# synthesizer-project/synference

Hardware: AMD Instinct MI355X
Metric: posterior samples/sec (accepted, prior-box rejection included) (higher is better)
Workload: dtype f32

## Files before the change

include/synference_hip.h:

```cpp
#ifndef SYNFERENCE_HIP_H
#define SYNFERENCE_HIP_H

#include <stddef.h>
#include <stdint.h>

#ifdef __cplusplus
extern "C" {
#endif

typedef struct sf_flow sf_flow;
typedef struct sf_opt sf_opt;

enum sf_status {
  SF_OK = 0,
  SF_ERR_INVALID = -1,
  SF_ERR_HIP = -2,
  SF_ERR_NO_DEVICE = -3,
  SF_ERR_STATE = -4
};

enum sf_kind { SF_MAF = 0, SF_NSF = 1, SF_NSF_AR = 2, SF_MAF_AR = 3 };

typedef struct sf_flow_desc {
  int32_t kind;
// ... 23 lines not shown
void sf_flow_destroy(sf_flow* f);
int64_t sf_flow_num_params(const sf_flow* f);
int64_t sf_flow_packed_size(const sf_flow* f);

int sf_flow_set_params(sf_flow* f, const float* flat, int64_t n, int is_device, void* stream);

int sf_flow_get_params(sf_flow* f, float* flat, int64_t n, int is_device, void* stream);

int sf_flow_pack_table(const sf_flow* f, int32_t* src1, int32_t* src2, int64_t n_packed);
int64_t sf_flow_packed16_size(const sf_flow* f);
int sf_flow_pack_table16(const sf_flow* f, int32_t* src1, int32_t* src2, int64_t n_packed16);
int64_t sf_flow_packed16b_size(const sf_flow* f);
int sf_flow_pack_table16b(const sf_flow* f, int32_t* src, int64_t n);
int64_t sf_flow_packed16c_size(const sf_flow* f);
int sf_flow_pack_table16c(const sf_flow* f, int32_t* src, int64_t n);
int64_t sf_flow_trainc_size(const sf_flow* f);
int64_t sf_flow_trainc_grad_size(const sf_flow* f);
int sf_flow_trainc_table(const sf_flow* f, int32_t* src1, int32_t* src2, int64_t n, int32_t* gdst, int64_t n_params,
                         int32_t* desc , float* cst, int64_t n_cst);
int64_t sf_flow_cst_size(const sf_flow* f);
int sf_flow_train_path(const sf_flow* f, int64_t B, int want_dctx);
int sf_flow_describe(const sf_flow* f, char* buf, size_t buflen);

int sf_flow_log_prob(sf_flow* f, const float* theta , const float* x ,
                     int64_t B, float* out , void* stream);

int sf_flow_log_prob_grad(sf_flow* f, const float* theta , const float* x, int64_t rows_per_x, int64_t B,
                          float* lp , float* dtheta , void* stream);

int sf_map_step(int64_t B, int64_t D, float* phi , float* exp_avg , float* exp_avg_sq ,
// ... 272 lines not shown
```

synference_amd/_lib.py:

```python
from __future__ import annotations

import ctypes as C
import os
from pathlib import Path

_HERE = Path(__file__).resolve().parent
LIB_PATH = _HERE / "lib" / "libsynference_hip.so"

c_f32p = C.POINTER(C.c_float)
c_i32p = C.POINTER(C.c_int32)
c_u32p = C.POINTER(C.c_uint32)


class sf_flow_desc(C.Structure):
    _fields_ = [
        ("kind", C.c_int32), ("D", C.c_int32), ("C", C.c_int32), ("H", C.c_int32),
        ("T", C.c_int32), ("K", C.c_int32), ("NB", C.c_int32), ("scale_fn", C.c_int32),
        ("hidden_bf16", C.c_int32),
        ("tail_bound", C.c_float), ("min_bin_width", C.c_float), ("min_bin_height", C.c_float),
        ("min_derivative", C.c_float), ("maf_eps", C.c_float), ("lu_eps", C.c_float),
        ("theta_mean", c_f32p), ("theta_std", c_f32p), ("x_mean", c_f32p), ("x_std", c_f32p),
        ("perms", c_i32p), ("ar_slope", C.c_float),
    ]

# ... 69 lines not shown
    "sf_flow_packed16_size": (C.c_int64, [C.c_void_p]),
    "sf_flow_pack_table16": (C.c_int, [C.c_void_p, C.c_void_p, C.c_void_p, C.c_int64]),
    "sf_flow_packed16b_size": (C.c_int64, [C.c_void_p]),
    "sf_flow_inverse_from_noise_sampler": (C.c_int, [C.c_void_p, C.c_void_p, C.c_void_p, C.c_int64, C.c_void_p, C.c_void_p]),
    "sf_set_sampler_fp32": (C.c_int, [C.c_int]),
    "sf_flow_set_sample_row_offset": (C.c_int, [C.c_void_p, C.c_int64]),
    "sf_flow_train_path": (C.c_int, [C.c_void_p, C.c_int64, C.c_int]),
    "sf_flow_trainc_size": (C.c_int64, [C.c_void_p]),
    "sf_flow_trainc_grad_size": (C.c_int64, [C.c_void_p]),
    "sf_flow_cst_size": (C.c_int64, [C.c_void_p]),
    "sf_flow_trainc_table": (C.c_int, [C.c_void_p, C.c_void_p, C.c_void_p, C.c_int64, C.c_void_p, C.c_int64, C.c_void_p,
                                       C.c_void_p, C.c_int64]),
    "sf_flow_pack_table16b": (C.c_int, [C.c_void_p, C.c_void_p, C.c_int64]),
    "sf_flow_packed16c_size": (C.c_int64, [C.c_void_p]),
    "sf_flow_pack_table16c": (C.c_int, [C.c_void_p, C.c_void_p, C.c_int64]),
    "sf_flow_get_params": (C.c_int, [C.c_void_p, C.c_void_p, C.c_int64, C.c_int, C.c_void_p]),
    "sf_flow_prepare_context": (C.c_int, [C.c_void_p, C.c_void_p, C.c_int64, C.c_void_p]),
    "sf_flow_release_context": (C.c_int, [C.c_void_p]),
    "sf_flow_sample": (C.c_int, [C.c_void_p, C.c_void_p, C.c_int64, C.c_int64, C.c_void_p, C.c_void_p,
                                 C.c_uint64, C.c_int32, C.c_void_p, C.c_void_p, C.POINTER(C.c_int64),
                                 C.c_void_p]),
    "sf_flow_sample_slots": (C.c_int, [C.c_void_p, C.c_void_p, C.c_int64, C.c_int64, C.c_void_p, C.c_int64, C.c_void_p,
                                       C.c_void_p, C.c_uint64, C.c_int32, C.c_void_p, C.POINTER(C.c_int64), C.c_void_p]),
    "sf_flow_sample_stats": (C.c_int, [C.c_void_p, C.POINTER(C.c_float)]),
    "sf_flow_acceptance": (C.c_int, [C.c_void_p, C.c_void_p, C.c_int64, C.c_int64, C.c_void_p, C.c_void_p,
                                     C.c_uint64, C.c_void_p, C.c_void_p]),
    "sf_flow_loss_grad": (C.c_int, [C.c_void_p, C.c_void_p, C.c_void_p, C.c_void_p, C.c_int64, C.c_float,
                                    C.c_void_p, C.c_void_p, C.c_void_p]),
    "sf_flow_loss_grad_rows": (C.c_int, [C.c_void_p, C.c_void_p, C.c_void_p, C.c_void_p, C.c_void_p, C.c_int64,
                                         C.c_float, C.c_void_p, C.c_void_p, C.c_void_p, C.c_void_p, C.c_void_p,
# ... 92 lines not shown
```

synference_amd/csrc/sf_api.hip:

```cpp
#include <hip/hip_runtime.h>

#include <chrono>
#include <cmath>
#include <cstdio>
#include <cstdlib>
#include <cstring>
#include <string>
#include <vector>

#include "sf_internal.h"
#include "sf_train.h"
#include "sf_nsf1.h"
#include "sf_nsfar.h"
#include "sf_nsfc.h"
#include "sf_trainc.h"

namespace {
thread_local std::string g_err;

int hip_fail(hipError_t e, const char* what) {
  return sf_fail(SF_ERR_HIP, std::string(what) + ": " + hipGetErrorString(e));
}
}

// ... 14 lines not shown
  SF_TRY_SET(hipMemset(d.d_packed, 0, np * sizeof(float)));
  SF_TRY_SET(d.d_cst.upload(f->L.cst));
  SF_TRY_SET(d.d_s1.alloc(np));
  SF_TRY_SET(d.d_s2.alloc(np));
  SF_TRY_SET(hipMemcpy(d.d_s1, f->L.src1.data(), np * sizeof(int32_t), hipMemcpyHostToDevice));
  SF_TRY_SET(hipMemcpy(d.d_s2, f->L.src2.data(), np * sizeof(int32_t), hipMemcpyHostToDevice));
  if ((f->L.dev.m16_ok || f->L.nsfS.ok) && f->L.n_packed16 > 0) {
    const size_t n16 = (size_t)f->L.n_packed16;
    SF_TRY_SET(d.d_packed16.alloc(n16));
    SF_TRY_SET(d.d_s16a.alloc(n16));
    SF_TRY_SET(d.d_s16b.alloc(n16));
    SF_TRY_SET(hipMemcpy(d.d_s16a, f->L.src16a.data(), n16 * sizeof(int32_t), hipMemcpyHostToDevice));
    SF_TRY_SET(hipMemcpy(d.d_s16b, f->L.src16b.data(), n16 * sizeof(int32_t), hipMemcpyHostToDevice));
  }
  if (f->L.dev.m16_ok && f->L.n_packed16 > 0 && sf_maf16_compact_fix(f->L.dev) == 1) {
    SF_TRY_SET(d.d_packed16c.alloc((size_t)f->L.dev.t16c_stride * f->L.dev.T));
    SF_TRY_SET(d.d_s16c.upload(f->L.src16c));
  }
  if ((f->L.dev.m16_ok || f->L.nsfS.ok) && f->L.n_packed16B > 0) {
    const size_t nB = (size_t)f->L.n_packed16B;
    SF_TRY_SET(d.d_packed16B.alloc(nB));
    SF_TRY_SET(d.d_s16B.alloc(nB));
    SF_TRY_SET(hipMemcpy(d.d_s16B, f->L.src16B.data(), nB * sizeof(int32_t), hipMemcpyHostToDevice));
  }
  if (f->L.n_packedB > 0) {
    SF_TRY_SET(d.d_packedB.alloc((size_t)f->L.n_packedB));
    SF_TRY_SET(d.d_bsrc.alloc((size_t)f->L.n_packedB));
    SF_TRY_SET(hipMemcpy(d.d_bsrc, f->L.srcB.data(), (size_t)f->L.n_packedB * sizeof(int32_t), hipMemcpyHostToDevice));
  }
  SF_TRY_SET(d.d_flat.alloc((size_t)f->L.n_params));
  SF_TRY_SET(d.d_cnt.alloc(SF_MAX_ROUNDS));
  SF_TRY_SET(d.h_cnt.alloc(SF_MAX_ROUNDS));
// ... 94 lines not shown
int64_t sf_flow_packed16b_size(const sf_flow* f) { return (f && f->L.dev.m16_ok) ? f->L.n_packed16B : 0; }

int sf_flow_pack_table16b(const sf_flow* f, int32_t* src, int64_t n) {
  if (!f || !src) return sf_fail(SF_ERR_INVALID, "null argument");
  if (!f->L.dev.m16_ok || n != f->L.n_packed16B) return sf_fail(SF_ERR_INVALID, "no split-bf16 image or size mismatch");
  std::memcpy(src, f->L.src16B.data(), (size_t)n * sizeof(int32_t));
  return SF_OK;
}

int64_t sf_flow_packed16c_size(const sf_flow* f) { return (f && f->L.dev.m16_ok) ? (int64_t)f->L.src16c.size() : 0; }

int sf_flow_pack_table16c(const sf_flow* f, int32_t* src, int64_t n) {
  if (!f || !src) return sf_fail(SF_ERR_INVALID, "null argument");
  if (!f->L.dev.m16_ok || n == 0 || n != (int64_t)f->L.src16c.size()) return sf_fail(SF_ERR_INVALID, "no compact fused image or size mismatch");
  std::memcpy(src, f->L.src16c.data(), (size_t)n * sizeof(int32_t));
  return SF_OK;
}

int64_t sf_flow_trainc_size(const sf_flow* f) { return (f && (f->L.trc.ok || f->L.nsc.ok)) ? f->L.n_imgC : 0; }
int64_t sf_flow_trainc_grad_size(const sf_flow* f) { return (f && (f->L.trc.ok || f->L.nsc.ok)) ? f->L.n_gradC : 0; }
int64_t sf_flow_cst_size(const sf_flow* f) { return f ? (int64_t)f->L.cst.size() : 0; }
int sf_flow_trainc_table(const sf_flow* f, int32_t* src1, int32_t* src2, int64_t n, int32_t* gdst, int64_t n_params,
                         int32_t* desc, float* cst, int64_t n_cst) {
  if (!f || !src1 || !src2 || !gdst || !desc || !cst) return sf_fail(SF_ERR_INVALID, "null argument");
  if ((!f->L.trc.ok && !f->L.nsc.ok) || n != f->L.n_imgC || n_params != f->L.n_params || n_cst != (int64_t)f->L.cst.size())
    return sf_fail(SF_ERR_INVALID, "no cooperative training image or size mismatch");
  static_assert(sizeof(SfTrcDev) <= 64 * sizeof(int32_t) && sizeof(SfNscDev) <= 64 * sizeof(int32_t), "descriptor words");
  std::memcpy(src1, f->L.srcC1.data(), (size_t)n * sizeof(int32_t));
  std::memcpy(src2, f->L.srcC2.data(), (size_t)n * sizeof(int32_t));
  std::memcpy(gdst, f->L.gdstC.data(), (size_t)n_params * sizeof(int32_t));
// ... 46 lines not shown
  add("inc_ok", v.inc_ok); add("hidden_bf16", v.hidden_bf16); add("tB_stride", v.tB_stride); add("n_parts", v.n_parts); add("part_max", v.part_max);
  add("n_params", f->L.n_params); add("n_packed", f->L.n_packed);
  {
    int R = 0, NV = 0;
    SfDev vv = v;
    vv.packed16 = reinterpret_cast<const float*>(1);
    sf_ctab_shape(vv, R, NV);
    add("ctab_floats_per_galaxy", (long)v.T * NV * R);
  }
  add("o16_w0", v.o16_w0); add("o16_wc", v.o16_wc); add("o16_b0", v.o16_b0); add("o16_wk0", v.o16_wk[0]);
  add("o16_wk1", v.o16_wk[1]); add("o16_bk0", v.o16_bk[0]); add("o16_bk1", v.o16_bk[1]); add("o16_hv", v.o16_hv);
  add("o16_hvb", v.o16_hvb); add("o16_wh", v.o16_wh); add("o16_bh", v.o16_bh); add("o16_wp", v.o16_wp); add("t16_a_tab", v.t16_a_tab);
  add("t16_a", v.t16_a); add("t16B_stride", v.t16B_stride); add("nP16", v.nP16); add("o16B_wk0", v.o16B_wk[0]); add("o16B_wk1", v.o16B_wk[1]);
  add("t16c_stride", v.t16c_stride); add("o16c_bk1", v.o16c_bk1); add("o16c_hvb", v.o16c_hvb); add("o16c_bh", v.o16c_bh);
  add("o16c_wh", v.o16c_wh); add("o16c_wp", v.o16c_wp); add("o16c_blk", v.o16c_blk); add("c16_fix", sf_maf16_compact_fix(v));
  add("sampler_fused", (f->dev_ready && f->ctab_x) ? (sf_maf16_plan(sampler_dev(f, f->ctab_x)).fused ? 1 : 0) : 0);
  add("m16_ok", v.m16_ok); add("m16_span", v.m16_span); add("m16_k3", v.m16_k3); add("nT16", v.nT16); add("nC16", v.nC16); add("t16_stride", v.t16_stride);
  s += "\"g16_tile\": [";
  for (int i = 0; i < SF_DMAX; ++i) s += std::to_string(v.g16_tile[i]) + (i + 1 < SF_DMAX ? ", " : "], ");
  s += "\"g16_lo\": [";
  for (int i = 0; i < SF_DMAX; ++i) s += std::to_string(v.g16_lo[i]) + (i + 1 < SF_DMAX ? ", " : "], ");
  s += "\"g_kend\": [";
  for (int i = 0; i < SF_DMAX; ++i) s += std::to_string(v.g_kend[i]) + (i + 1 < SF_DMAX ? ", " : "], ");
  s += "\"g_lo\": [";
  for (int i = 0; i < SF_DMAX; ++i) s += std::to_string(v.g_lo[i]) + (i + 1 < SF_DMAX ? ", " : "], ");
  s += "\"g_tile\": [";
  for (int i = 0; i < SF_DMAX; ++i) s += std::to_string(v.g_tile[i]) + (i + 1 < SF_DMAX ? ", " : "], ");
  s += "\"mt_kend\": [";
  for (int i = 0; i < 4; ++i) s += std::to_string(v.mt_kend[i]) + (i + 1 < 4 ? ", " : "], ");
  s += "\"cst\": [";
// ... 812 lines not shown
```

synference_amd/csrc/sf_layout.cpp:

```cpp
#include "sf_layout.h"

#include <cmath>
#include <cstring>
#include <functional>

namespace {

struct Emitter {
  std::vector<int32_t>& s1;
  std::vector<int32_t>& s2;
  std::vector<int32_t>* gidx = nullptr;
  int64_t cur = 0;

  int64_t pad_to(int64_t align) {
    while (cur % align) push(-1, -1);
    return cur;
  }
  void push(int32_t a, int32_t b, int64_t g = -1) {
    s1.push_back(a);
    s2.push_back(b);
    if (gidx) gidx->push_back((int32_t)(g >= 0 ? g : cur));
    ++cur;
  }
  int64_t linear(int OT, int nG, const std::vector<int>& orow, const std::vector<int>& irow,
// ... 999 lines not shown
    run(v.o16_hvb, 2 * D);
    align(4);
    v.o16c_bh = here();
    run(v.o16_bh, 16);
    v.o16c_wh = here();
    run(v.o16_wh, NT * 256);
    v.o16c_wp = here();
    const int KN = std::min(NT, D - 1);
    run(v.o16_wp, (KN * NT - KN * (KN - 1) / 2) * 16);
    v.o16c_blk = here();
    if (NB == 2)
      for (int ot = 0; ot < NT; ++ot)
        for (int it = 0; it <= ot; ++it) run(v.o16_wk[1] + (ot * NT + it) * 256, 256);
    align(256);
    v.t16c_stride = here();
  }
  L.n_packedB = (int64_t)L.srcB.size();
  {
    const int budget = 152 * 1024 / 4;
    std::vector<int> cuts;
    if (d.kind == SF_MAF) {
      cuts = {0, v.t_stride};
    } else {
      cuts.push_back(0);
      for (int k = 0; k < NB; ++k) cuts.push_back(v.o_wg[k]);
      cuts.push_back(v.o_wout);
      cuts.push_back(v.t_stride);
    }
    v.n_parts = 0;
    v.part_max = 0;
// ... 102 lines not shown
```

synference_amd/csrc/sf_layout.h:

```cpp
#pragma once
#include <cstdint>
#include <string>
#include <vector>

#include "../../include/synference_hip.h"

#define SF_DMAX 16
#define SF_NBMAX 4

struct SfDev {
  const float* packed;
  const float* packedT;
  const float* cst;
  int kind, D, C, H, T, K, NB, scale_fn;
  int HT;
  int PT;
  int KMAX;
  int JP;
  int nGu, nGc, nGh;
  int t_stride;
  int n_parts, part_off[5], part_max;
  int blk_part[SF_NBMAX], head_part;
  int partB_off[5], part_bytes_max;
  int o_w0, o_wc, o_b0;
// ... 15 lines not shown
  int g_tile[SF_DMAX], g_kend[SF_DMAX];
  int g_lo[SF_DMAX];
  int mt_kend[4];
  const unsigned short* packedB;
  int hidden_bf16, nKS, tB_stride;
  int oB_wk[SF_NBMAX], oB_w1[SF_NBMAX], oB_w2[SF_NBMAX];
  const float* packed16;
  int m16_ok, nT16, nC16, t16_stride;
  int t16_a;
  int t16_a_tab;
  int o16_wh, o16_bh;
  int o16_wp;
  const float* packed16c;
  int t16c_stride;
  int o16c_bk1, o16c_hvb, o16c_bh, o16c_wh, o16c_wp, o16c_blk;
  const uint32_t* packed16B;
  int t16B_stride, nP16, o16B_wk[2];
  int m16_span;
  int m16_k3;
  int o16_w0, o16_wc, o16_b0, o16_wk[2], o16_bk[2], o16_hv, o16_hvb;
  int g16_tile[SF_DMAX];
  int g16_lo[SF_DMAX];
  const float* ctab;
  int ctab_R, ctab_NV;
  int c_pscale, c_pshift, c_tdim, c_xmean, c_xstd;
  int c_dslot;
  float logdet0;
  float tail_bound, min_w, min_h, min_d, eps, lu_eps, inv_sqrt_h, deriv_const;
};

// ... 42 lines not shown
  std::vector<int32_t> srcC1, srcC2;
  std::vector<int32_t> gdstC;
  int64_t n_imgC = 0, n_gradC = 0;
  int64_t n_params = 0;
  int64_t n_packed = 0;
  std::vector<int32_t> src1, src2;
  std::vector<int32_t> srcT1, srcT2;
  int64_t n_packedT = 0;
  std::vector<int32_t> gdst;
  std::vector<int32_t> srcB;
  std::vector<int32_t> src16a, src16b;
  std::vector<int32_t> src16B;
  int64_t n_packed16B = 0;
  int64_t n_packed16 = 0;
  std::vector<int32_t> src16c;
  int64_t n_packedB = 0;
  std::vector<float> cst;
  std::string error;
};

static inline int sf_tile_row(int r, int h) { return (r & 3) + 8 * (r >> 2) + 4 * h; }

bool sf_build_layout(const sf_flow_desc& d, SfLayout& L);

#define SF_MLP_LMAX 4
struct SfMlpDev {
  const float* packed;
  const float* packedT;
  const float* cst;
  int n_in, n_out, L, act, HT;
// ... 14 lines not shown
```

synference_amd/csrc/sf_maf16.hip:

```cpp
#include "sf_maf16_pass.h"

template <int NB, bool SPAN>
__global__ __launch_bounds__(256, 3) void k_maf_inv16(SfDev m, SfSampleArgsHost a) {
  const int lane = threadIdx.x & 63, wave = threadIdx.x >> 6;
  const int s = lane & 15, g4 = lane >> 4;
  const long item = ((long)blockIdx.x * 4 + wave) * 16 + s;
  const bool valid = item < a.n_items;
  const long it = valid ? item : a.n_items - 1;
  const SfItem16 I = sf_item16(m, a, it, g4);
  f32x4 u = I.u;
  const uint32_t slot = I.slot, att_mine = I.att;
  const long gal = I.gal, ps_idx = I.ps;
  const float* xr = a.x + gal * m.C;
  float logdet = 0.f;

  const float* ctg = (m.ctab && !a.z_in) ? m.ctab + (size_t)gal * m.T * m.ctab_R : nullptr;
  f32x4 ct0;
  if (!ctg) ct0 = sf_ctx_tile16(m, xr, 0, g4);

  const int NT = m.nT16;
  SfPass16 S;
#pragma unroll
  for (int k = 0; k < 3; ++k)
#pragma unroll
// ... 123 lines not shown
           m.o16_hv == o_hv && m.o16_hvb == o_hvb && m.o16_wh == o_wh && m.o16_bh == o_bh && m.o16_wp == o_wp && m.t16_a_tab == a_tab &&
           m.o16B_wk[0] == 0 && (NB < 2 || m.o16B_wk[1] == oB_wk1) && m.t16B_stride == B_stride;
  }
  static __device__ __forceinline__ void apply(SfDev& m) {
    m.nT16 = NT; m.o16_w0 = o_w0; m.o16_b0 = o_b0; m.o16_bk[0] = o_bk0; m.o16_bk[1] = o_bk1; m.o16_hv = o_hv; m.o16_hvb = o_hvb;
    m.o16_wh = o_wh; m.o16_bh = o_bh; m.o16_wp = o_wp; m.t16_a_tab = a_tab; m.o16B_wk[0] = 0; m.o16B_wk[1] = oB_wk1; m.t16B_stride = B_stride;
  }
};

template <int NB, int DD>
struct SfFixC16 {
  static constexpr int NT = DD - 1, ENT = NT * (NT + 1) / 2;
  static constexpr int o_bk1 = 0, o_hvb = NB == 2 ? NT * 16 : 0, o_bh = o_hvb + (2 * DD + 3) / 4 * 4, o_wh = o_bh + 16;
  static constexpr int o_wp = o_wh + NT * 256, o_blk = o_wp + ENT * 16;
  static constexpr int size = (o_blk + (NB == 2 ? ENT * 256 : 0) + 255) / 256 * 256;
  static constexpr int groups = size / 256;
  static bool matches(const SfDev& m) {
    return m.nT16 == NT && m.o16c_bk1 == o_bk1 && m.o16c_hvb == o_hvb && m.o16c_bh == o_bh && m.o16c_wh == o_wh && m.o16c_wp == o_wp &&
           m.o16c_blk == o_blk && m.t16c_stride == size;
  }
  static __device__ __forceinline__ void apply(SfDev& m) {
    m.o16_bk[1] = o_bk1; m.o16_hvb = o_hvb; m.o16_bh = o_bh; m.o16_wh = o_wh; m.o16_wp = o_wp;
  }
};
template <int PREC>
static __host__ __device__ __forceinline__ int sf_lds_floats16(const SfDev& m, bool cp) {
  if constexpr (PREC == 2) return m.t16c_stride + 4 * SF_G16_SCR;
  else return (m.ctab ? m.t16_a_tab : m.t16_a) + SfHid16<PREC>::lds_floats(m, cp);
}
template <int G>
__device__ __forceinline__ void sf_stage16c(const float* src, int wave) {
  const float4* __restrict__ g = reinterpret_cast<const float4*>(src) + (threadIdx.x & 63);
  float4* __restrict__ l = reinterpret_cast<float4*>(sf_lds16);
  for (int gi = __builtin_amdgcn_readfirstlane(wave); gi < G; gi += 4)
    __builtin_amdgcn_global_load_lds((const void*)(g + gi * 64), (void __attribute__((address_space(3)))*)(l + gi * 64), 16, 0, 0);
  __builtin_amdgcn_s_waitcnt(0x0f70);
}

#ifndef SF_SAMP16_WG_FUSED
#define SF_SAMP16_WG_FUSED 4
#endif
template <int NB, bool SPAN, bool HM, int DD = 0, int PREC = 0, int K3 = 0>
__global__ __launch_bounds__(256, (SPAN ? 3 : (PREC == 2 ? SF_SAMP16_WG_FUSED : 4))) void k_maf_samp16(SfSamp16Args args_in) {
  static_assert(K3 == 0 || (PREC == 2 && K3 <= DD - 1), "skipped k-steps: the fused passes only, at most every hidden tile");
  static_assert(DD == 0 || (HM && !SPAN && DD >= 2 && DD <= 5), "unrolled passes: head tile, aligned placement, D <= 5");
  static_assert(PREC != 2 || DD >= 3, "fused first layer: unrolled kernels only (m_fix and the compact image's offsets)");
  using HID = SfHid16<PREC>;
  constexpr int TPW = SF_SAMP16_TPW;
  constexpr int IPW = 64 * TPW;
  const int wave = threadIdx.x >> 6;
  using FC = SfFixC16<NB, (PREC == 2 ? DD : 2)>;
  unsigned int* ctrl = reinterpret_cast<unsigned int*>(sf_lds16 + sf_lds_floats16<PREC>(args_in.m, !SPAN));
  unsigned int pf;
  sf_q_begin<IPW>(args_in.a, ctrl, pf);
  float* ecb = reinterpret_cast<float*>(ctrl + SF_Q_WORDS(IPW));
  sf_ecb16_build<true>(ecb, args_in.m, args_in.a);
#ifdef SF_Q_STATS
  const unsigned long long qs_k0 = __builtin_amdgcn_s_memtime();
  unsigned long long qs_iters = 0, qs_last_work = 0;
  unsigned long long qs_ph[10] = {0, 0, 0, 0, 0, 0, 0, 0, 0, 0};
  if (threadIdx.x == 0) atomicMin(&args_in.a.q->stats[10], __builtin_amdgcn_s_memrealtime());
#endif
  for (;;) {
    const SfSamp16Args* ap;
    {
      auto kp = __builtin_amdgcn_kernarg_segment_ptr();
      asm volatile("" : "+s"(kp));
// ... 55 lines not shown
      g_t[j] = slot / (uint32_t)a.S;
    }
    SfTiles16 tiles;
    if constexpr (DD == 0) tiles.pack(m);
    typename HID::State S;
    S.tab = DD > 0 ? true : m.ctab != nullptr;
    for (int t = m.T - 1; t >= 0; --t) {
      const int dsl = (int)m.cst[m.c_dslot + t * SF_DMAX + s];
      S.c0p = S.tab ? m.ctab + ((size_t)gal_cur * m.T + t) * m.ctab_R + (PREC == 2 ? m.nT16 * 16 : 0) : nullptr;
      if constexpr (PREC == 2) sf_pre16g_load<DD - 1>(S, g4);
      else if (HM && S.tab) sf_c0_prefetch(S, tiles.tile(2), g4);
#ifdef SF_Q_STATS
      { const unsigned long long n = __builtin_amdgcn_s_memrealtime(); qs_ph[qs_o + (t == m.T - 1 ? 1 : 3)] += n - qs_t_mark; qs_t_mark = n; }
#endif
      __syncthreads();
      if constexpr (PREC == 2) sf_stage16c<FC::groups>(m.packed16c + (size_t)t * FC::size, wave);
      else sf_stage16<PREC, !SPAN>(m, t, S.tab ? m.t16_a_tab : m.t16_a, wave);
      __syncthreads();
#ifdef SF_Q_STATS
      { const unsigned long long n = __builtin_amdgcn_s_memrealtime(); qs_ph[qs_o + 2] += n - qs_t_mark; qs_t_mark = n; }
#endif
      const float* tp = sf_lds16;
      const void* tpB = sf_lds16 + (PREC == 2 ? FC::o_blk : (S.tab ? m.t16_a_tab : m.t16_a));
#pragma unroll 1
      for (int j = 0; j < TPW; ++j) {
        const bool tile_has_work = (unsigned)((j * 4 + wave) * 16) < n_items;
        if (tile_has_work) {
          if (j > 0) {
            S.c0p = S.tab ? m.ctab + ((size_t)gal_cur * m.T + t) * m.ctab_R + (PREC == 2 ? m.nT16 * 16 : 0) : nullptr;
            if constexpr (PREC == 2) sf_pre16g_load<DD - 1>(S, g4);
            else if (HM && S.tab) sf_c0_prefetch(S, tiles.tile(2), g4);
          }
          if (HM) S.hdone = sf_ld4(tp + m.o16_bh + g4 * 4);
          if constexpr (PREC == 2) {
            float* scr = sf_lds16 + FC::size + wave * SF_G16_SCR + s * SF_G16_ROW;
            sf_transform16g<NB, DD, K3>(m, tp, static_cast<const float*>(tpB), S, dsl, u_cur, scr, lane, g4);
          } else {
            S.xr = a.x + gal_cur * m.C;
            if constexpr (DD > 0) {
              sf_transform16s<HID, NB, DD>(m, tp, tpB, S, NT, dsl, u_cur, lane, g4);
            } else {
              HID::template clear<false, HM>(S);
#pragma unroll
              for (int r = 0; r < 4; ++r) S.ut[r] = 0.f;
              {
                const int sl = __builtin_amdgcn_readlane(dsl, 0);
                sf_pass16_deg1(m, tp, S.ut, sl, sf_slot16_own(u_cur, sl), g4);
              }
              for (int p = 2; p <= m.D; ++p) {
                const int sl = __builtin_amdgcn_readlane(dsl, p - 1);
                sf_pass16_tiles<HID, NB, SPAN, HM>(m, tp, tpB, S, NT, tiles, p, m.D, sl, sf_slot16_own(u_cur, sl), lane, g4);
// ... 109 lines not shown
    qs_ph[qs_o + 4] += qs_last_work - qs_t_mark;
    if (a.qtrace && threadIdx.x == 0 && qs_iters <= (2048u * 256u) / gridDim.x)
      a.qtrace[((size_t)blockIdx.x * ((2048u * 256u) / gridDim.x) + qs_iters - 1) * 4 + 3] = (uint32_t)qs_last_work;
#endif
  }
}

template <int NB, int DD, int PREC = 0, int K3 = 0>
__global__ __launch_bounds__(256, 4) void k_maf_find16s(SfDev m, SfSampleArgsHost a) {
  static_assert(K3 == 0 || (PREC == 2 && K3 <= DD - 1), "skipped k-steps: the fused passes only");
  using HID = SfHid16<PREC>;
  using FC = SfFixC16<NB, DD>;
  SfFix16<NB, DD>::apply(m);
  const int lane = threadIdx.x & 63, wave = threadIdx.x >> 6;
  const int s = lane & 15, g4 = lane >> 4;
  float* ecb = sf_lds16 + sf_lds_floats16<PREC>(m, true);
  sf_ecb16_build<false>(ecb, m, a);
  if constexpr (PREC == 2) FC::apply(m);
  const int NT = m.nT16;
  f32x4 u_cur, u_oth;
  long gal_cur = 0, gal_oth = 0;
#pragma unroll
  for (int j = 1; j >= 0; --j) {
    const long item = ((long)blockIdx.x * 8 + j * 4 + wave) * 16 + s;
    const long it = item < a.n_items ? item : a.n_items - 1;
    const SfItem16 I = sf_item16(m, a, it, g4);
    if (j == 1) { u_oth = I.u; gal_oth = I.gal; }
    else { u_cur = I.u; gal_cur = I.gal; }
  }
  typename HID::State S;
  S.tab = true;
  if constexpr (PREC != 2) S.xr = nullptr;
  for (int t = m.T - 1; t >= 0; --t) {
    const int dsl = (int)m.cst[m.c_dslot + t * SF_DMAX + s];
    S.c0p = m.ctab + ((size_t)gal_cur * m.T + t) * m.ctab_R + (PREC == 2 ? m.nT16 * 16 : 0);
    if constexpr (PREC == 2) sf_pre16g_load<DD - 1>(S, g4);
    else sf_c0_prefetch(S, 0, g4);
    __syncthreads();
    if constexpr (PREC == 2) sf_stage16c<FC::groups>(m.packed16c + (size_t)t * FC::size, wave);
    else sf_stage16<PREC, true>(m, t, m.t16_a_tab, wave);
    __syncthreads();
    const float* tp = sf_lds16;
    const void* tpB = sf_lds16 + (PREC == 2 ? FC::o_blk : m.t16_a_tab);
#pragma unroll 1
    for (int j = 0; j < 2; ++j) {
      if (((long)blockIdx.x * 8 + j * 4 + wave) * 16 < a.n_items) {
        if (j > 0) {
          S.c0p = m.ctab + ((size_t)gal_cur * m.T + t) * m.ctab_R + (PREC == 2 ? m.nT16 * 16 : 0);
          if constexpr (PREC == 2) sf_pre16g_load<DD - 1>(S, g4);
          else sf_c0_prefetch(S, 0, g4);
        }
        S.hdone = sf_ld4(tp + m.o16_bh + g4 * 4);
        if constexpr (PREC == 2) {
          float* scr = sf_lds16 + FC::size + wave * SF_G16_SCR + s * SF_G16_ROW;
          sf_transform16g<NB, DD, K3>(m, tp, static_cast<const float*>(tpB), S, dsl, u_cur, scr, lane, g4);
        } else {
          sf_transform16s<HID, NB, DD>(m, tp, tpB, S, NT, dsl, u_cur, lane, g4);
        }
      }
      { const f32x4 tu = u_cur; u_cur = u_oth; u_oth = tu; }
      { const long tg = gal_cur; gal_cur = gal_oth; gal_oth = tg; }
    }
  }
#pragma unroll 1
  for (int j = 0; j < 2; ++j) {
    const long item = ((long)blockIdx.x * 8 + j * 4 + wave) * 16 + s;
    const bool valid = item < a.n_items;
    const long it = valid ? item : a.n_items - 1;
    const long ps = it >> a.log2_attempts;
    const uint32_t att = a.att_list ? a.att_list[ps] : a.attempt + (uint32_t)(it & ((1L << a.log2_attempts) - 1));
// ... 240 lines not shown
    double acc = 0.0;
    for (int it = 0; it < NT; ++it)
      for (int kk = 0; kk < 16; ++kk) {
        const float wk = tp[m.o16_wk[0] + ((ot * NT + it) * 64 + row + 16 * (kk >> 2)) * 4 + (kk & 3)];
        const float w0 = tp[m.o16_w0 + (it * 64 + kk + 16 * (col >> 2)) * 4 + (col & 3)];
        acc += (double)wk * (double)w0;
      }
    tp[m.o16_wp + e * 16 + g4 * 4 + r] = (float)acc;
  }
}
hipError_t sf_launch_maf_fuse16(const SfDev& m, hipStream_t st) {
  hipLaunchKernelGGL(k_maf_fuse16, dim3((unsigned)m.T), dim3(256), 0, st, m);
  return hipGetLastError();
}
__global__ __launch_bounds__(256) void k_maf_compact16(SfDev m, const int32_t* __restrict__ tab, float* __restrict__ out) {
  const float* tp = m.packed16 + (size_t)blockIdx.x * m.t16_stride;
  float* op = out + (size_t)blockIdx.x * m.t16c_stride;
  for (int i = threadIdx.x; i < m.t16c_stride; i += blockDim.x) {
    const int s = tab[i];
    op[i] = s >= 0 ? tp[s] : 0.f;
  }
}
hipError_t sf_launch_maf_compact16(const SfDev& m, const int32_t* tab, float* out, hipStream_t st) {
  hipLaunchKernelGGL(k_maf_compact16, dim3((unsigned)m.T), dim3(256), 0, st, m, tab, out);
  return hipGetLastError();
}
hipError_t sf_launch_maf_ctab16(const SfDev& m, const float* x, long M, float* tab, hipStream_t st) {
  hipLaunchKernelGGL(k_maf_ctab16, dim3((unsigned)((M + 63) / 64), (unsigned)m.T), dim3(256), 0, st, m, x, M, tab);
  return hipGetLastError();
}

bool sf_maf16_enabled(const SfDev& m, const SfSampleArgsHost& a) {
  return sf_maf16_plan(m).ok16 && (a.attempts_per_slot <= 16 || a.best != nullptr);
}
// ... 74 lines not shown
```

synference_amd/csrc/sf_maf16_pass.h:

```cpp
#pragma once
#include <hip/hip_runtime.h>

#include <type_traits>

#include "sf_device.h"
#include "sf_internal.h"
#include "sf_rng.h"

typedef float f32x4 __attribute__((ext_vector_type(4)));
typedef float f32x2 __attribute__((ext_vector_type(2)));
#define SF_MFMA16(a, b, c) __builtin_amdgcn_mfma_f32_16x16x4f32((a), (b), (c), 0, 0, 0)

__device__ __forceinline__ float sf_sum4groups(float v) {
  v += __shfl_xor(v, 16, 64);
  v += __shfl_xor(v, 32, 64);
  return v;
}
__device__ __forceinline__ f32x4 sf_mma16(float4 w, const f32x4& in, f32x4 acc) {
  acc = SF_MFMA16(w.x, in[0], acc);
  acc = SF_MFMA16(w.y, in[1], acc);
  acc = SF_MFMA16(w.z, in[2], acc);
  acc = SF_MFMA16(w.w, in[3], acc);
  return acc;
}
// ... 514 lines not shown
#pragma unroll
      for (int ot = 0; ot < 4; ++ot)
#pragma unroll
        for (int r = 0; r < 4; ++r) S.head[ot][r] = 0.f;
    }
  }
  static __host__ __device__ int lds_floats(const SfDev& m, bool cp) {
    const int nb = m.NB < 2 ? m.NB : 2;
    return nb * (cp ? m.nT16 * (m.nT16 + 1) / 2 : m.nT16 * m.nT16) * 256;
  }
};

struct SfPass16G {
  f32x4 act[4];
  f32x4 pre[4];
  f32x4 hdone;
  const float* c0p;
  bool tab;
};
__host__ __device__ constexpr int sf_wp16_entry(int NT, int k, int ot) { return (k - 1) * NT - (k - 1) * (k - 2) / 2 + ot - (k - 1); }
#define SF_G16_ROW 20
#define SF_G16_SCR (16 * SF_G16_ROW)
template <int NT>
__device__ __forceinline__ void sf_pre16g_load(SfPass16G& S, int g4) {
#pragma unroll
  for (int ot = 0; ot < NT; ++ot) S.pre[ot] = *reinterpret_cast<const f32x4*>(S.c0p + ot * 16 + 4 * g4);
}
__device__ __forceinline__ f32x4 sf_rank1(const f32x4& acc, const float4& w, float v) {
  const f32x2 vv = {v, v};
  const f32x2 lo = __builtin_elementwise_fma(f32x2{w.x, w.y}, vv, f32x2{acc[0], acc[1]});
  const f32x2 hi = __builtin_elementwise_fma(f32x2{w.z, w.w}, vv, f32x2{acc[2], acc[3]});
  return f32x4{lo[0], lo[1], hi[0], hi[1]};
}
template <int NT, int K>
struct SfWpCols {
  float4 w[NT - K + 1];
  __device__ __forceinline__ void load(const float* tp, int o_wp, int g4) {
#pragma unroll
    for (int q = 0; q <= NT - K; ++q) w[q] = *reinterpret_cast<const float4*>(tp + o_wp + sf_wp16_entry(NT, K, K - 1 + q) * 16 + 4 * g4);
  }
  __device__ __forceinline__ void apply(SfPass16G& S, float wv) const {
#pragma unroll
    for (int q = 0; q <= NT - K; ++q) S.pre[K - 1 + q] = sf_rank1(S.pre[K - 1 + q], w[q], wv);
  }
};
template <bool SKIP>
__device__ __forceinline__ f32x4 sf_mma16k(float4 w, const f32x4& in, f32x4 acc) {
  acc = SF_MFMA16(w.x, in[0], acc);
  acc = SF_MFMA16(w.y, in[1], acc);
  acc = SF_MFMA16(w.z, in[2], acc);
  if constexpr (!SKIP) acc = SF_MFMA16(w.w, in[3], acc);
  return acc;
}
template <bool SKIP>
__device__ __forceinline__ f32x4 sf_tanh4k(const f32x4& b) {
  if constexpr (!SKIP) {
    return sf_tanh4(b);
  } else {
    const f32x2 one = {1.0f, 1.0f}, m2 = {-2.0f, -2.0f};
    const f32x2 e01 = f32x2{__builtin_amdgcn_exp2f(b[0]), __builtin_amdgcn_exp2f(b[1])} + one;
    const float e2 = __builtin_amdgcn_exp2f(b[2]) + 1.0f;
    const f32x2 r01 = {__builtin_amdgcn_rcpf(e01[0]), __builtin_amdgcn_rcpf(e01[1])};
    const f32x2 o01 = __builtin_elementwise_fma(r01, m2, one);
    return f32x4{o01[0], o01[1], __builtin_fmaf(__builtin_amdgcn_rcpf(e2), -2.0f, 1.0f), 0.f};
  }
}
template <int OT, int NB, int NT, int K3 = 0>
__device__ __forceinline__ float sf_pass16g(const SfDev& m, const float* tp, const float* tpF, SfPass16G& S, int sl, float u_in,
                                            int lane, int g4) {
  constexpr bool SK = OT >= NT - K3;
  const float4 wh = sf_w16(tp + m.o16_wh, NT, 0, OT, lane);
  float4 fw[OT + 1];
  f32x4 b1;
  if (NB == 2) {
    b1 = sf_ld4(tp + m.o16_bk[1] + (OT * 4 + g4) * 4);
#pragma unroll
    for (int it = 0; it <= OT; ++it) fw[it] = sf_w16f<true>(tpF, NT, OT, it, lane);
  }
  SfWpCols<NT, (OT + 2 <= NT ? OT + 2 : NT)> wu;
  if constexpr (OT + 2 <= NT) wu.load(tp, m.o16_wp, g4);
  __builtin_amdgcn_sched_barrier(0);
  if (NB == 2) {
#pragma unroll
    for (int it = 0; it < OT; ++it) b1 = it >= NT - K3 ? sf_mma16k<true>(fw[it], S.act[it], b1) : sf_mma16k<false>(fw[it], S.act[it], b1);
  }
  f32x4 last = sf_tanh4k<SK>(S.pre[OT]);
  if (NB == 2) {
    S.act[OT] = last;
    b1 = sf_mma16k<SK>(fw[OT], last, b1);
    last = sf_tanh4k<SK>(b1);
  }
  S.hdone = sf_mma16k<SK>(wh, last, S.hdone);
  const bool odd = (sl & 1) != 0;
  const int src = (lane & 15) + 16 * (sl >> 1);
  const float av = __shfl(odd ? S.hdone[2] : S.hdone[0], src, 64);
  const float mv = __shfl(odd ? S.hdone[3] : S.hdone[1], src, 64);
  const float wv = sf_div(u_in - mv, sf_scale16(m, av));
  if constexpr (OT + 2 <= NT) wu.apply(S, wv);
  return wv;
}
template <int NB, int DD, int K3 = 0>
__device__ __forceinline__ void sf_transform16g(const SfDev& m, const float* tp, const float* tpF, SfPass16G& S, int dsl, f32x4& u,
                                                float* scr, int lane, int g4) {
  constexpr int NT = DD - 1;
  *reinterpret_cast<f32x4*>(scr + 4 * g4) = u;
  int sl[DD];
  float ud[DD];
#pragma unroll
  for (int q = 0; q < DD; ++q) {
    sl[q] = __builtin_amdgcn_readlane(dsl, q);
    ud[q] = scr[sl[q]];
  }
  {
    SfWpCols<NT, 1> wu;
    wu.load(tp, m.o16_wp, g4);
    const float av = tp[m.o16_hvb + 2 * sl[0]], mv = tp[m.o16_hvb + 2 * sl[0] + 1];
    const float wv = sf_div(ud[0] - mv, sf_scale16(m, av));
    wu.apply(S, wv);
    scr[sl[0]] = wv;
  }
  auto pass = [&](auto otc) {
    constexpr int OT = decltype(otc)::value;
    scr[sl[OT + 1]] = sf_pass16g<OT, NB, NT, K3>(m, tp, tpF, S, sl[OT + 1], ud[OT + 1], lane, g4);
  };
  pass(std::integral_constant<int, 0>{});
  if constexpr (DD >= 3) pass(std::integral_constant<int, 1>{});
  if constexpr (DD >= 4) pass(std::integral_constant<int, 2>{});
  if constexpr (DD >= 5) pass(std::integral_constant<int, 3>{});
  u = *reinterpret_cast<const f32x4*>(scr + 4 * g4);
}
template <> struct SfHid16<2> {
  using State = SfPass16G;
};

__device__ __forceinline__ void sf_copy_group16(const float4* g, float4* l) {
  __builtin_amdgcn_global_load_lds((const void*)g, (void __attribute__((address_space(3)))*)l, 16, 0, 0);
  __builtin_amdgcn_global_load_lds((const void*)g, (void __attribute__((address_space(3)))*)l, 16, 1024, 0);
  __builtin_amdgcn_global_load_lds((const void*)g, (void __attribute__((address_space(3)))*)l, 16, 2048, 0);
// ... 157 lines not shown
```

synference_amd/engine.py:

```python
from __future__ import annotations

import ctypes as C
import json
from typing import Optional, Tuple

import numpy as np
import torch

from . import _lib
from .spec import KIND_ID, FlowSpec, num_params


def retry_width(pending: int, attempt: int, max_attempts: int, total: int = 0) -> int:
    A = 1
    if attempt > 0:
        budget = 262144
        while A < 16 and 2 * A * pending <= budget and attempt + 2 * A <= max_attempts:
            A *= 2
    return A


def _ptr(t: Optional[torch.Tensor]):
    return None if t is None else C.c_void_p(t.data_ptr())

# ... 61 lines not shown
        return s1, s2

    def pack_table16b(self) -> np.ndarray:
        n = int(self.lib.sf_flow_packed16b_size(self.handle))
        s = np.empty(n, np.int32)
        if n:
            _lib.check(self.lib.sf_flow_pack_table16b(self.handle, s.ctypes.data_as(_lib.c_i32p), n))
        return s

    def pack_table16c(self) -> np.ndarray:
        n = int(self.lib.sf_flow_packed16c_size(self.handle))
        s = np.empty(n, np.int32)
        if n:
            _lib.check(self.lib.sf_flow_pack_table16c(self.handle, s.ctypes.data_as(_lib.c_i32p), n))
        return s

    TRC_FIELDS = ("ok NT NI t_stride g_stride o_win o_b0 o_w1 o_b1 o_w2 o_b2 o_wf o_bf o_wfT o_w2T o_w1T o_winT "
                  "g_win g_b0 g_w1 g_b1 g_w2 g_b2 g_wf g_bf kend0 kend1 kend2 kend3 kbeg0 kbeg1 kbeg2 kbeg3 c_insrc c_jobs "
                  "n_jobs").split()

    NSC_FIELDS = ("ok NT NI OTQ KM kc_h kc_in0 kc_in1 kc_in2 t_stride g_stride o_win o_bin o_wg0 o_wg1 o_bg0 o_bg1 o_w10 o_w11 "
                  "o_b10 o_b11 o_w20 o_w21 o_b20 o_b21 o_wout o_bout o_lu o_woutT o_w2T0 o_w2T1 o_w1T0 o_w1T1 o_winT "
                  "g_win g_bin g_wg0 g_wg1 g_bg0 g_bg1 g_w10 g_w11 g_b10 g_b11 g_w20 g_w21 g_b20 g_b21 g_wout g_bout g_lu").split()

    def trainc_table(self):
        n = int(self.lib.sf_flow_trainc_size(self.handle))
        if not n:
            return None
        s1 = np.empty(n, np.int32)
        s2 = np.empty(n, np.int32)
# ... 239 lines not shown
```

Before: 1.164 billion.

## Replace MMA-based MAF head with per-transform head-row table and FMA accumulation

Adds a per-transform head-row region to the compact fused parameter image, holding the masked hidden-to-output weights for each later output dimension, permuted by sigma. The sampler pass now accumulates output-head partial sums incrementally with FMAs as each hidden tile becomes available, instead of a 16x16 MMA plus two cross-lane shuffles per output. Staging skips the now-unused wh/bh groups in LDS. This trades an MMA and shuffles for extra LDS reads, cross-group reductions and more LDS footprint per block, which may reduce occupancy.

```diff
diff --git a/include/synference_hip.h b/include/synference_hip.h
--- a/include/synference_hip.h
+++ b/include/synference_hip.h
@@ -61,6 +61,8 @@
 int sf_flow_pack_table16b(const sf_flow* f, int32_t* src, int64_t n);
 int64_t sf_flow_packed16c_size(const sf_flow* f);
 int sf_flow_pack_table16c(const sf_flow* f, int32_t* src, int64_t n);
+int64_t sf_flow_packed16h_size(const sf_flow* f);
+int sf_flow_pack_table16h(const sf_flow* f, int32_t* src, int64_t n);
 int64_t sf_flow_trainc_size(const sf_flow* f);
 int64_t sf_flow_trainc_grad_size(const sf_flow* f);
 int sf_flow_trainc_table(const sf_flow* f, int32_t* src1, int32_t* src2, int64_t n, int32_t* gdst, int64_t n_params,
diff --git a/synference_amd/_lib.py b/synference_amd/_lib.py
--- a/synference_amd/_lib.py
+++ b/synference_amd/_lib.py
@@ -107,6 +107,8 @@
     "sf_flow_pack_table16b": (C.c_int, [C.c_void_p, C.c_void_p, C.c_int64]),
     "sf_flow_packed16c_size": (C.c_int64, [C.c_void_p]),
     "sf_flow_pack_table16c": (C.c_int, [C.c_void_p, C.c_void_p, C.c_int64]),
+    "sf_flow_packed16h_size": (C.c_int64, [C.c_void_p]),
+    "sf_flow_pack_table16h": (C.c_int, [C.c_void_p, C.c_void_p, C.c_int64]),
     "sf_flow_get_params": (C.c_int, [C.c_void_p, C.c_void_p, C.c_int64, C.c_int, C.c_void_p]),
     "sf_flow_prepare_context": (C.c_int, [C.c_void_p, C.c_void_p, C.c_int64, C.c_void_p]),
     "sf_flow_release_context": (C.c_int, [C.c_void_p]),
diff --git a/synference_amd/csrc/sf_api.hip b/synference_amd/csrc/sf_api.hip
--- a/synference_amd/csrc/sf_api.hip
+++ b/synference_amd/csrc/sf_api.hip
@@ -52,8 +52,14 @@
     SF_TRY_SET(hipMemcpy(d.d_s16b, f->L.src16b.data(), n16 * sizeof(int32_t), hipMemcpyHostToDevice));
   }
   if (f->L.dev.m16_ok && f->L.n_packed16 > 0 && sf_maf16_compact_fix(f->L.dev) == 1) {
-    SF_TRY_SET(d.d_packed16c.alloc((size_t)f->L.dev.t16c_stride * f->L.dev.T));
-    SF_TRY_SET(d.d_s16c.upload(f->L.src16c));
+    const SfDev& v = f->L.dev;
+    SF_TRY_SET(d.d_packed16c.alloc((size_t)(v.t16c_stride + v.t16h_stride) * v.T));
+    std::vector<int32_t> tab;
+    for (int t = 0; t < v.T; ++t) {
+      tab.insert(tab.end(), f->L.src16c.begin(), f->L.src16c.end());
+      tab.insert(tab.end(), f->L.src16h.begin() + (size_t)t * v.t16h_stride, f->L.src16h.begin() + (size_t)(t + 1) * v.t16h_stride);
+    }
+    SF_TRY_SET(d.d_s16c.upload(tab));
   }
   if ((f->L.dev.m16_ok || f->L.nsfS.ok) && f->L.n_packed16B > 0) {
     const size_t nB = (size_t)f->L.n_packed16B;
@@ -178,6 +184,15 @@
   if (!f || !src) return sf_fail(SF_ERR_INVALID, "null argument");
   if (!f->L.dev.m16_ok || n == 0 || n != (int64_t)f->L.src16c.size()) return sf_fail(SF_ERR_INVALID, "no compact fused image or size mismatch");
   std::memcpy(src, f->L.src16c.data(), (size_t)n * sizeof(int32_t));
+  return SF_OK;
+}
+
+int64_t sf_flow_packed16h_size(const sf_flow* f) { return (f && f->L.dev.m16_ok) ? (int64_t)f->L.src16h.size() : 0; }
+
+int sf_flow_pack_table16h(const sf_flow* f, int32_t* src, int64_t n) {
+  if (!f || !src) return sf_fail(SF_ERR_INVALID, "null argument");
+  if (!f->L.dev.m16_ok || n == 0 || n != (int64_t)f->L.src16h.size()) return sf_fail(SF_ERR_INVALID, "no head-row region or size mismatch");
+  std::memcpy(src, f->L.src16h.data(), (size_t)n * sizeof(int32_t));
   return SF_OK;
 }
 
@@ -254,6 +269,7 @@
   add("t16_a", v.t16_a); add("t16B_stride", v.t16B_stride); add("nP16", v.nP16); add("o16B_wk0", v.o16B_wk[0]); add("o16B_wk1", v.o16B_wk[1]);
   add("t16c_stride", v.t16c_stride); add("o16c_bk1", v.o16c_bk1); add("o16c_hvb", v.o16c_hvb); add("o16c_bh", v.o16c_bh);
   add("o16c_wh", v.o16c_wh); add("o16c_wp", v.o16c_wp); add("o16c_blk", v.o16c_blk); add("c16_fix", sf_maf16_compact_fix(v));
+  add("t16h_stride", v.t16h_stride);
   add("sampler_fused", (f->dev_ready && f->ctab_x) ? (sf_maf16_plan(sampler_dev(f, f->ctab_x)).fused ? 1 : 0) : 0);
   add("m16_ok", v.m16_ok); add("m16_span", v.m16_span); add("m16_k3", v.m16_k3); add("nT16", v.nT16); add("nC16", v.nC16); add("t16_stride", v.t16_stride);
   s += "\"g16_tile\": [";
diff --git a/synference_amd/csrc/sf_layout.cpp b/synference_amd/csrc/sf_layout.cpp
--- a/synference_amd/csrc/sf_layout.cpp
+++ b/synference_amd/csrc/sf_layout.cpp
@@ -1037,6 +1037,17 @@
         for (int it = 0; it <= ot; ++it) run(v.o16_wk[1] + (ot * NT + it) * 256, 256);
     align(256);
     v.t16c_stride = here();
+    const int NE = D * (D - 1) / 2;
+    v.t16h_stride = (NE * 32 + 255) / 256 * 256;
+    L.src16h.assign((size_t)T * v.t16h_stride, -1);
+    for (int t = 0; t < T; ++t) {
+      int32_t* th = L.src16h.data() + (size_t)t * v.t16h_stride;
+      int e = 0;
+      for (int ot = 0; ot < NT; ++ot)
+        for (int k = ot + 2; k <= D; ++k, ++e)
+          for (int g4 = 0; g4 < 4; ++g4)
+            for (int i = 0; i < 8; ++i) th[e * 32 + g4 * 8 + i] = v.o16_hv + sigma[t][k - 1] * 128 + g4 * 32 + ot * 8 + i;
+    }
   }
   L.n_packedB = (int64_t)L.srcB.size();
   {
diff --git a/synference_amd/csrc/sf_layout.h b/synference_amd/csrc/sf_layout.h
--- a/synference_amd/csrc/sf_layout.h
+++ b/synference_amd/csrc/sf_layout.h
@@ -53,6 +53,7 @@
   const float* packed16c;
   int t16c_stride;
   int o16c_bk1, o16c_hvb, o16c_bh, o16c_wh, o16c_wp, o16c_blk;
+  int t16h_stride;
   const uint32_t* packed16B;
   int t16B_stride, nP16, o16B_wk[2];
   int m16_span;
@@ -125,6 +126,7 @@
   int64_t n_packed16B = 0;
   int64_t n_packed16 = 0;
   std::vector<int32_t> src16c;
+  std::vector<int32_t> src16h;
   int64_t n_packedB = 0;
   std::vector<float> cst;
   std::string error;
diff --git a/synference_amd/csrc/sf_maf16.hip b/synference_amd/csrc/sf_maf16.hip
--- a/synference_amd/csrc/sf_maf16.hip
+++ b/synference_amd/csrc/sf_maf16.hip
@@ -161,26 +161,31 @@
   static constexpr int o_bk1 = 0, o_hvb = NB == 2 ? NT * 16 : 0, o_bh = o_hvb + (2 * DD + 3) / 4 * 4, o_wh = o_bh + 16;
   static constexpr int o_wp = o_wh + NT * 256, o_blk = o_wp + ENT * 16;
   static constexpr int size = (o_blk + (NB == 2 ? ENT * 256 : 0) + 255) / 256 * 256;
-  static constexpr int groups = size / 256;
+  static constexpr int o_hr = size, hr_size = (sf_hr16_entries(DD) * 32 + 255) / 256 * 256, total = size + hr_size;
+  static constexpr int lds = total + 4 * SF_G16_SCR;
+  static constexpr int groups = total / 256, dead_lo = (o_bh + 255) / 256, dead_hi = o_wp / 256;
   static bool matches(const SfDev& m) {
     return m.nT16 == NT && m.o16c_bk1 == o_bk1 && m.o16c_hvb == o_hvb && m.o16c_bh == o_bh && m.o16c_wh == o_wh && m.o16c_wp == o_wp &&
-           m.o16c_blk == o_blk && m.t16c_stride == size;
+           m.o16c_blk == o_blk && m.t16c_stride == size && m.t16h_stride == hr_size;
   }
   static __device__ __forceinline__ void apply(SfDev& m) {
-    m.o16_bk[1] = o_bk1; m.o16_hvb = o_hvb; m.o16_bh = o_bh; m.o16_wh = o_wh; m.o16_wp = o_wp;
+    m.o16_bk[1] = o_bk1; m.o16_hvb = o_hvb; m.o16_wp = o_wp;
   }
 };
 template <int PREC>
 static __host__ __device__ __forceinline__ int sf_lds_floats16(const SfDev& m, bool cp) {
-  if constexpr (PREC == 2) return m.t16c_stride + 4 * SF_G16_SCR;
+  if constexpr (PREC == 2) return m.t16c_stride + m.t16h_stride + 4 * SF_G16_SCR;
   else return (m.ctab ? m.t16_a_tab : m.t16_a) + SfHid16<PREC>::lds_floats(m, cp);
 }
-template <int G>
+template <int G, int DEAD_LO = 0, int DEAD_HI = 0>
 __device__ __forceinline__ void sf_stage16c(const float* src, int wave) {
   const float4* __restrict__ g = reinterpret_cast<const float4*>(src) + (threadIdx.x & 63);
   float4* __restrict__ l = reinterpret_cast<float4*>(sf_lds16);
-  for (int gi = __builtin_amdgcn_readfirstlane(wave); gi < G; gi += 4)
+  constexpr int ND = DEAD_HI > DEAD_LO ? DEAD_HI - DEAD_LO : 0;
+  for (int q = __builtin_amdgcn_readfirstlane(wave); q < G - ND; q += 4) {
+    const int gi = q < DEAD_LO ? q : q + ND;
     __builtin_amdgcn_global_load_lds((const void*)(g + gi * 64), (void __attribute__((address_space(3)))*)(l + gi * 64), 16, 0, 0);
+  }
   __builtin_amdgcn_s_waitcnt(0x0f70);
 }
 
@@ -197,7 +202,7 @@
   constexpr int IPW = 64 * TPW;
   const int wave = threadIdx.x >> 6;
   using FC = SfFixC16<NB, (PREC == 2 ? DD : 2)>;
-  unsigned int* ctrl = reinterpret_cast<unsigned int*>(sf_lds16 + sf_lds_floats16<PREC>(args_in.m, !SPAN));
+  unsigned int* ctrl = reinterpret_cast<unsigned int*>(sf_lds16 + (PREC == 2 ? FC::lds : sf_lds_floats16<PREC>(args_in.m, !SPAN)));
   unsigned int pf;
   sf_q_begin<IPW>(args_in.a, ctrl, pf);
   float* ecb = reinterpret_cast<float*>(ctrl + SF_Q_WORDS(IPW));
@@ -283,7 +288,7 @@
       { const unsigned long long n = __builtin_amdgcn_s_memrealtime(); qs_ph[qs_o + (t == m.T - 1 ? 1 : 3)] += n - qs_t_mark; qs_t_mark = n; }
 #endif
       __syncthreads();
-      if constexpr (PREC == 2) sf_stage16c<FC::groups>(m.packed16c + (size_t)t * FC::size, wave);
+      if constexpr (PREC == 2) sf_stage16c<FC::groups, FC::dead_lo, FC::dead_hi>(m.packed16c + (size_t)t * FC::total, wave);
       else sf_stage16<PREC, !SPAN>(m, t, S.tab ? m.t16_a_tab : m.t16_a, wave);
       __syncthreads();
 #ifdef SF_Q_STATS
@@ -300,10 +305,10 @@
             if constexpr (PREC == 2) sf_pre16g_load<DD - 1>(S, g4);
             else if (HM && S.tab) sf_c0_prefetch(S, tiles.tile(2), g4);
           }
-          if (HM) S.hdone = sf_ld4(tp + m.o16_bh + g4 * 4);
+          if constexpr (PREC != 2) { if (HM) S.hdone = sf_ld4(tp + m.o16_bh + g4 * 4); }
           if constexpr (PREC == 2) {
-            float* scr = sf_lds16 + FC::size + wave * SF_G16_SCR + s * SF_G16_ROW;
-            sf_transform16g<NB, DD, K3>(m, tp, static_cast<const float*>(tpB), S, dsl, u_cur, scr, lane, g4);
+            float* scr = sf_lds16 + FC::total + wave * SF_G16_SCR + s * SF_G16_ROW;
+            sf_transform16g<NB, DD, K3>(m, tp, static_cast<const float*>(tpB), tp + FC::o_hr, S, dsl, u_cur, scr, lane, g4);
           } else {
             S.xr = a.x + gal_cur * m.C;
             if constexpr (DD > 0) {
@@ -443,7 +448,7 @@
   SfFix16<NB, DD>::apply(m);
   const int lane = threadIdx.x & 63, wave = threadIdx.x >> 6;
   const int s = lane & 15, g4 = lane >> 4;
-  float* ecb = sf_lds16 + sf_lds_floats16<PREC>(m, true);
+  float* ecb = sf_lds16 + (PREC == 2 ? FC::lds : sf_lds_floats16<PREC>(m, true));
   sf_ecb16_build<false>(ecb, m, a);
   if constexpr (PREC == 2) FC::apply(m);
   const int NT = m.nT16;
@@ -466,7 +471,7 @@
     if constexpr (PREC == 2) sf_pre16g_load<DD - 1>(S, g4);
     else sf_c0_prefetch(S, 0, g4);
     __syncthreads();
-    if constexpr (PREC == 2) sf_stage16c<FC::groups>(m.packed16c + (size_t)t * FC::size, wave);
+    if constexpr (PREC == 2) sf_stage16c<FC::groups, FC::dead_lo, FC::dead_hi>(m.packed16c + (size_t)t * FC::total, wave);
     else sf_stage16<PREC, true>(m, t, m.t16_a_tab, wave);
     __syncthreads();
     const float* tp = sf_lds16;
@@ -479,10 +484,10 @@
           if constexpr (PREC == 2) sf_pre16g_load<DD - 1>(S, g4);
           else sf_c0_prefetch(S, 0, g4);
         }
-        S.hdone = sf_ld4(tp + m.o16_bh + g4 * 4);
+        if constexpr (PREC != 2) S.hdone = sf_ld4(tp + m.o16_bh + g4 * 4);
         if constexpr (PREC == 2) {
-          float* scr = sf_lds16 + FC::size + wave * SF_G16_SCR + s * SF_G16_ROW;
-          sf_transform16g<NB, DD, K3>(m, tp, static_cast<const float*>(tpB), S, dsl, u_cur, scr, lane, g4);
+          float* scr = sf_lds16 + FC::total + wave * SF_G16_SCR + s * SF_G16_ROW;
+          sf_transform16g<NB, DD, K3>(m, tp, static_cast<const float*>(tpB), tp + FC::o_hr, S, dsl, u_cur, scr, lane, g4);
         } else {
           sf_transform16s<HID, NB, DD>(m, tp, tpB, S, NT, dsl, u_cur, lane, g4);
         }
@@ -753,10 +758,12 @@
   return hipGetLastError();
 }
 __global__ __launch_bounds__(256) void k_maf_compact16(SfDev m, const int32_t* __restrict__ tab, float* __restrict__ out) {
+  const int n = m.t16c_stride + m.t16h_stride;
   const float* tp = m.packed16 + (size_t)blockIdx.x * m.t16_stride;
-  float* op = out + (size_t)blockIdx.x * m.t16c_stride;
-  for (int i = threadIdx.x; i < m.t16c_stride; i += blockDim.x) {
-    const int s = tab[i];
+  const int32_t* tt = tab + (size_t)blockIdx.x * n;
+  float* op = out + (size_t)blockIdx.x * n;
+  for (int i = threadIdx.x; i < n; i += blockDim.x) {
+    const int s = tt[i];
     op[i] = s >= 0 ? tp[s] : 0.f;
   }
 }
diff --git a/synference_amd/csrc/sf_maf16_pass.h b/synference_amd/csrc/sf_maf16_pass.h
--- a/synference_amd/csrc/sf_maf16_pass.h
+++ b/synference_amd/csrc/sf_maf16_pass.h
@@ -552,10 +552,20 @@
 struct SfPass16G {
   f32x4 act[4];
   f32x4 pre[4];
-  f32x4 hdone;
+  f32x2 ham[4];
   const float* c0p;
   bool tab;
 };
+__host__ __device__ constexpr int sf_hr16_entry(int D, int ot, int k) { return ot * (D - 1) - ot * (ot - 1) / 2 + (k - ot - 2); }
+__host__ __device__ constexpr int sf_hr16_entries(int D) { return D * (D - 1) / 2; }
+template <bool SKIP>
+__device__ __forceinline__ f32x2 sf_head_acck(f32x2 acc, const float4& h01, const float4& h23, const f32x4& v) {
+  acc = __builtin_elementwise_fma(f32x2{h01.x, h01.y}, f32x2{v[0], v[0]}, acc);
+  acc = __builtin_elementwise_fma(f32x2{h01.z, h01.w}, f32x2{v[1], v[1]}, acc);
+  acc = __builtin_elementwise_fma(f32x2{h23.x, h23.y}, f32x2{v[2], v[2]}, acc);
+  if constexpr (!SKIP) acc = __builtin_elementwise_fma(f32x2{h23.z, h23.w}, f32x2{v[3], v[3]}, acc);
+  return acc;
+}
 __host__ __device__ constexpr int sf_wp16_entry(int NT, int k, int ot) { return (k - 1) * NT - (k - 1) * (k - 2) / 2 + ot - (k - 1); }
 #define SF_G16_ROW 20
 #define SF_G16_SCR (16 * SF_G16_ROW)
@@ -579,7 +589,10 @@
   }
   __device__ __forceinline__ void apply(SfPass16G& S, float wv) const {
 #pragma unroll
-    for (int q = 0; q <= NT - K; ++q) S.pre[K - 1 + q] = sf_rank1(S.pre[K - 1 + q], w[q], wv);
+    for (int q = 0; q <= NT - K; ++q) {
+      S.pre[K - 1 + q] = sf_rank1(S.pre[K - 1 + q], w[q], wv);
+      if (q > 0) asm volatile("" : "+v"(S.pre[K - 1 + q]));
+    }
   }
 };
 template <bool SKIP>
@@ -604,10 +617,20 @@
   }
 }
 template <int OT, int NB, int NT, int K3 = 0>
-__device__ __forceinline__ float sf_pass16g(const SfDev& m, const float* tp, const float* tpF, SfPass16G& S, int sl, float u_in,
-                                            int lane, int g4) {
+__device__ __forceinline__ float sf_pass16g(const SfDev& m, const float* tp, const float* tpF, const float* hr, SfPass16G& S, int sl,
+                                            const float* scr, int lane, int g4) {
   constexpr bool SK = OT >= NT - K3;
-  const float4 wh = sf_w16(tp + m.o16_wh, NT, 0, OT, lane);
+  constexpr int D = NT + 1, NH = D - (OT + 1);
+  float4 h01[NH], h23[NH];
+#pragma unroll
+  for (int q = 0; q < NH; ++q) {
+    const float* p = hr + sf_hr16_entry(D, OT, OT + 2 + q) * 32 + g4 * 8;
+    h01[q] = *reinterpret_cast<const float4*>(p);
+    if constexpr (SK) { const float2 t = *reinterpret_cast<const float2*>(p + 4); h23[q] = float4{t.x, t.y, 0.f, 0.f}; }
+    else h23[q] = *reinterpret_cast<const float4*>(p + 4);
+  }
+  const float ba = tp[m.o16_hvb + 2 * sl], bm = tp[m.o16_hvb + 2 * sl + 1];
+  const float u_in = scr[sl];
   float4 fw[OT + 1];
   f32x4 b1;
   if (NB == 2) {
@@ -628,38 +651,40 @@
     b1 = sf_mma16k<SK>(fw[OT], last, b1);
     last = sf_tanh4k<SK>(b1);
   }
-  S.hdone = sf_mma16k<SK>(wh, last, S.hdone);
-  const bool odd = (sl & 1) != 0;
-  const int src = (lane & 15) + 16 * (sl >> 1);
-  const float av = __shfl(odd ? S.hdone[2] : S.hdone[0], src, 64);
-  const float mv = __shfl(odd ? S.hdone[3] : S.hdone[1], src, 64);
+  const f32x2 pam = sf_head_acck<SK>(S.ham[OT], h01[0], h23[0], last);
+  const float sa = sf_sum4groups(pam[0]), sm = sf_sum4groups(pam[1]);
+#pragma unroll
+  for (int q = 1; q < NH; ++q) {
+    S.ham[OT + q] = sf_head_acck<SK>(S.ham[OT + q], h01[q], h23[q], last);
+    asm volatile("" : "+v"(S.ham[OT + q]));
+  }
+  const float av = ba + sa, mv = bm + sm;
   const float wv = sf_div(u_in - mv, sf_scale16(m, av));
   if constexpr (OT + 2 <= NT) wu.apply(S, wv);
   return wv;
 }
 template <int NB, int DD, int K3 = 0>
-__device__ __forceinline__ void sf_transform16g(const SfDev& m, const float* tp, const float* tpF, SfPass16G& S, int dsl, f32x4& u,
-                                                float* scr, int lane, int g4) {
+__device__ __forceinline__ void sf_transform16g(const SfDev& m, const float* tp, const float* tpF, const float* hr, SfPass16G& S,
+                                                int dsl, f32x4& u, float* scr, int lane, int g4) {
   constexpr int NT = DD - 1;
+#pragma unroll
+  for (int q = 0; q < NT; ++q) S.ham[q] = f32x2{0.f, 0.f};
   *reinterpret_cast<f32x4*>(scr + 4 * g4) = u;
   int sl[DD];
-  float ud[DD];
-#pragma unroll
-  for (int q = 0; q < DD; ++q) {
-    sl[q] = __builtin_amdgcn_readlane(dsl, q);
-    ud[q] = scr[sl[q]];
-  }
+#pragma unroll
+  for (int q = 0; q < DD; ++q) sl[q] = __builtin_amdgcn_readlane(dsl, q);
   {
     SfWpCols<NT, 1> wu;
     wu.load(tp, m.o16_wp, g4);
     const float av = tp[m.o16_hvb + 2 * sl[0]], mv = tp[m.o16_hvb + 2 * sl[0] + 1];
-    const float wv = sf_div(ud[0] - mv, sf_scale16(m, av));
+    const float wv = sf_div(scr[sl[0]] - mv, sf_scale16(m, av));
     wu.apply(S, wv);
     scr[sl[0]] = wv;
   }
+  __builtin_amdgcn_sched_barrier(0);
   auto pass = [&](auto otc) {
     constexpr int OT = decltype(otc)::value;
-    scr[sl[OT + 1]] = sf_pass16g<OT, NB, NT, K3>(m, tp, tpF, S, sl[OT + 1], ud[OT + 1], lane, g4);
+    scr[sl[OT + 1]] = sf_pass16g<OT, NB, NT, K3>(m, tp, tpF, hr, S, sl[OT + 1], scr, lane, g4);
   };
   pass(std::integral_constant<int, 0>{});
   if constexpr (DD >= 3) pass(std::integral_constant<int, 1>{});
diff --git a/synference_amd/engine.py b/synference_amd/engine.py
--- a/synference_amd/engine.py
+++ b/synference_amd/engine.py
@@ -99,6 +99,13 @@
         if n:
             _lib.check(self.lib.sf_flow_pack_table16c(self.handle, s.ctypes.data_as(_lib.c_i32p), n))
         return s
+
+    def pack_table16h(self) -> np.ndarray:
+        n = int(self.lib.sf_flow_packed16h_size(self.handle))
+        s = np.empty(n, np.int32)
+        if n:
+            _lib.check(self.lib.sf_flow_pack_table16h(self.handle, s.ctypes.data_as(_lib.c_i32p), n))
+        return s.reshape(-1, self.describe()["t16h_stride"]) if n else s.reshape(0, 0)
 
     TRC_FIELDS = ("ok NT NI t_stride g_stride o_win o_b0 o_w1 o_b1 o_w2 o_b2 o_wf o_bf o_wfT o_w2T o_w1T o_winT "
                   "g_win g_b0 g_w1 g_b1 g_w2 g_b2 g_wf g_bf kend0 kend1 kend2 kend3 kbeg0 kbeg1 kbeg2 kbeg3 c_insrc c_jobs "
```

After: 1.238 billion (median of 6 runs). 1.06x the previous value.
